# seagochen/unet-segment-pytorch

Hardware: NVIDIA B200
Metric: AttentionUNet 512^2 train images/sec (whole job; per GPU = value / n_gpus) (higher is better)
Workload: dtype bf16

## Files before the change

### include/unetb200.h

```cpp
#ifndef UNETB200_H
#define UNETB200_H
#include <stddef.h>
#include <stdint.h>

#ifdef __cplusplus
extern "C" {
#endif

#define UB2_OK 0
#define UB2_ERR_SHAPE (-1)
#define UB2_ERR_ALIGN (-2)
#define UB2_ERR_WORKSPACE (-3)
#define UB2_ERR_DRIVER (-4)
#define UB2_ERR_ARCH (-5)

int ub2_version(void);
int ub2_num_sms(void);
int ub2_set_conv_mode(int mode);
int ub2_last_conv_variant(void);


int ub2_conv_fwd(const void* in0, int ld_in0, int C0, const void* in1, int ld_in1, int C1,
                 const void* wgt, void* out0, int ld0, void* out1, int ld1, int split, int N, int H,
                 int W, int Cout, int taps, const float* scale, const float* shift, int relu,
                 int accumulate, double* stats, int stats_rows, int* stats_rows_used,
                 int bn_override, int grid_override, void* stream);

int ub2_conv_wgrad(const void* in0, int ld_in0, int C0, const void* in1, int ld_in1, int C1,
                   const void* dy, int ld_dy, float* partial, int max_splits, int* splits_used,
                   int N, int H, int W, int Cout, int taps, int splits_override, void* stream);

int ub2_wgrad_reduce(float* partial, int splits, int Cout, int Cin, int taps, float* grad,
                     int accumulate, void* stream);

#define UB2_REDUCE_MAX_ITEMS 32
typedef struct Ub2ReduceItem {
  float* partial;
  float* grad;
  int splits, Cout, Cin, taps;
} Ub2ReduceItem;
int ub2_wgrad_reduce_multi(const Ub2ReduceItem* items, int n, int accumulate, void* stream);

int ub2_pack_conv_weight(const float* w, void* fwd, void* dgrad, int Cout, int Cin, int taps,
                         const float* out_scale, void* stream);
int ub2_pack_conv_weights_multi(const long long* desc, const int* blocks, int nblocks, void* stream);


int ub2_bn_finalize(const double* partials, int rows, int C, double count, const float* gamma,
                    const float* beta, float* running_mean, float* running_var, long long* nbt,
                    float momentum, float eps, float* scale, float* shift, float* mean, float* invstd,
                    void* stream);
int ub2_bn_eval_coeffs(const float* gamma, const float* beta, const float* running_mean,
                       const float* running_var, float eps, int C, float* scale, float* shift,
                       void* stream);
int ub2_bn_act(const void* y, int ld_y, const float* scale, const float* shift, void* a, int ld_a,
               void* pooled, int ld_p, unsigned char* pidx, int N, int H, int W, int C, int relu,
               void* stream);
int ub2_bn_bwd_rows(int N, int H, int W, int C, int pool);
int ub2_bn_bwd_reduce(const void* dA, int ld_da, const void* dP, int ld_dp, const unsigned char* pidx,
// ... 150 lines not shown
```

### unet-segment-pytorch_b200/csrc/capi_conv.cu

```cuda
#include "../../include/unetb200.h"
#include "conv.h"

using namespace ub2;

extern "C" {

int ub2_conv_fwd(const void* in0, int ld_in0, int C0, const void* in1, int ld_in1, int C1,
                 const void* wgt, void* out0, int ld0, void* out1, int ld1, int split, int N, int H,
                 int W, int Cout, int taps, const float* scale, const float* shift, int relu,
                 int accumulate, double* stats, int stats_rows, int* stats_rows_used,
                 int bn_override, int grid_override, void* stream) {
  ConvFwdArgs a{};
  a.in0 = in0; a.in1 = in1; a.wgt = wgt; a.out0 = out0; a.out1 = out1;
  a.scale = scale; a.shift = shift; a.stats = stats; a.grid_used = stats_rows_used;
  a.N = N; a.H = H; a.W = W; a.C0 = C0; a.C1 = C1; a.Cout = Cout; a.taps = taps;
  a.ld_in0 = ld_in0; a.ld_in1 = ld_in1; a.ld0 = ld0; a.ld1 = ld1; a.split = split;
  a.accumulate = accumulate; a.relu = relu; a.stats_rows = stats_rows;
  a.bn_override = bn_override; a.grid_override = grid_override;
  return conv_fwd_launch(a, static_cast<cudaStream_t>(stream));
}

int ub2_conv_fwd_tf32(const float* in0, int ld_in0, int C0, const float* in1, int ld_in1, int C1,
                      const float* wgt, float* out, int ld_out, int N, int H, int W, int Cout, int taps,
                      const float* scale, const float* shift, int relu, int exact_out, void* stream) {
  ConvFwdArgs a{};
  a.in0 = in0; a.in1 = in1; a.wgt = wgt; a.out0 = out;
  a.scale = scale; a.shift = shift; a.relu = relu;
  a.N = N; a.H = H; a.W = W; a.C0 = C0; a.C1 = C1; a.Cout = Cout; a.taps = taps;
  a.ld_in0 = ld_in0; a.ld_in1 = ld_in1; a.ld0 = ld_out;
  a.tf32 = exact_out ? 2 : 1;
  return conv_fwd_launch(a, static_cast<cudaStream_t>(stream));
}

int ub2_conv_wgrad(const void* in0, int ld_in0, int C0, const void* in1, int ld_in1, int C1,
                   const void* dy, int ld_dy, float* partial, int max_splits, int* splits_used,
                   int N, int H, int W, int Cout, int taps, int splits_override, void* stream) {
  ConvWgradArgs a{};
  a.in0 = in0; a.in1 = in1; a.dy = dy; a.partial = partial; a.splits_used = splits_used;
  a.N = N; a.H = H; a.W = W; a.C0 = C0; a.C1 = C1; a.Cout = Cout; a.taps = taps;
  a.ld_in0 = ld_in0; a.ld_in1 = ld_in1; a.ld_dy = ld_dy;
  a.max_splits = max_splits; a.splits_override = splits_override;
  return conv_wgrad_launch(a, static_cast<cudaStream_t>(stream));
}

int ub2_num_sms(void) { return num_sms(); }

int ub2_last_conv_variant(void) { return last_variant(); }

int ub2_set_conv_mode(int mode) {
  conv_set_mode(mode);
  return 0;
}

}
```

### unet-segment-pytorch_b200/csrc/conv.h

```cpp
#pragma once
#include <cuda.h>
#include <cuda_bf16.h>
#include <cuda_runtime.h>
#include <stddef.h>
#include <stdint.h>
#include <stdlib.h>

#define UB2_ERR_SHAPE (-1)
#define UB2_ERR_ALIGN (-2)
#define UB2_ERR_WORKSPACE (-3)
#define UB2_ERR_DRIVER (-4)
#define UB2_ERR_ARCH (-5)

namespace ub2 {

struct ConvFwdArgs {
  const void* in0;
  const void* in1;
  const void* wgt;
  void* out0;
  void* out1;
  const float* scale;
  const float* shift;
  double* stats;
  int* grid_used;
  int N, H, W, C0, C1, Cout, taps;
  int ld_in0, ld_in1, ld0, ld1, split;
  int accumulate, relu;
  int stats_rows;
  int bn_override, grid_override;
  int tf32;
};

struct ConvFwdParams {
  int N, H, W, C0, C1, Cout, taps, kc;
  int BW, BH, BI, tiles_w, tiles_h, tiles_n;
  int BN, n_tiles, stages, stage_bytes, tmem_cols;
  __nv_bfloat16* out0;
  __nv_bfloat16* out1;
  int ld0, ld1, split, accumulate, relu;
  int wide_store;
  int tf32;
  const float* scale;
  const float* shift;
  double* stats;
  int R, segs_w, blocks_h, a_bytes, b_stage_bytes, b_stages;
};

int conv_fwd_launch(const ConvFwdArgs& a, cudaStream_t stream);
int conv_halo_launch(const ConvFwdArgs& a, cudaStream_t stream);
void conv_set_mode(int mode);

struct ConvWgradArgs {
  const void* in0;
  const void* in1;
  const void* dy;
  float* partial;
  int* splits_used;
  int N, H, W, C0, C1, Cout, taps;
  int ld_in0, ld_in1, ld_dy;
  int max_splits;
  int splits_override;
};

struct ConvWgradParams {
  int N, H, W, C0, C1, Cout, taps, mc;
  int BW, BH, BI, chunks_w, chunks_h, chunks_n;
  int BN, n_tiles, m_tiles, splits, stages, stage_bytes, tmem_cols;
  int a_sub_bytes, b_sub_bytes, a_bytes;
  float* partial;
};

int conv_wgrad_launch(const ConvWgradArgs& a, cudaStream_t stream);

int make_tmap_nhwc(CUtensorMap* m, const void* base, int N, int H, int W, int C, int ld,
                   const uint32_t box[4], int swizzle_bytes, int elem_bytes = 2);
int make_tmap_2d(CUtensorMap* m, const void* base, uint64_t cols, uint64_t rows, uint64_t ld,
                 uint32_t bc, uint32_t br, int swizzle_bytes, int elem_bytes = 2);
int num_sms();
inline int cap_clusters(int occupancy_clusters) { const int c = num_sms() / 2; return occupancy_clusters < c ? occupancy_clusters : c; }
inline int wgrad_smem_budget() {
  static const int kb = [] { const char* e = getenv("UB2_WGRAD_SMEM_KB"); int v = e ? atoi(e) : 163; return v < 64 ? 64 : (v > 227 ? 227 : v); }();
  return kb * 1024;
// ... 19 lines not shown
```

### unet-segment-pytorch_b200/csrc/conv_fwd.cu

```cuda
#include "launch.cuh"
#include <cstdlib>
#include "conv.h"
#include "conv_epilogue.cuh"
#include "ptx.cuh"

namespace ub2 {

static constexpr int kMaxStages = 8;
static constexpr int kEpiWarps = 8;
static constexpr int kThreads = 64 + 32 * kEpiWarps;
static constexpr int kATileBytes = 128 * 64 * 2;

struct FwdSmemHeader {
  uint64_t full[kMaxStages];
  uint64_t empty[kMaxStages];
  uint64_t tmem_full[2];
  uint64_t tmem_empty[2];
  uint32_t tmem_base;
  uint32_t pad;
};

template <int TAPS, bool ACC, bool TF32>
__global__ void __launch_bounds__(kThreads, 1)
conv_fwd_kernel(const __grid_constant__ CUtensorMap tmA0, const __grid_constant__ CUtensorMap tmA1,
// ... 147 lines not shown
      const int as = it & 1;
      mbar_wait(&hdr->tmem_full[as], (it >> 1) & 1);
      tc_fence_after();
      for (int j = grp; j < nchunks; j += 2) {
        epi_chunk<ACC, TF32>(p, tmem_base + (static_cast<uint32_t>(q * 32) << 16) + as * bn_cols + j * 32,
                       n0 + j * 32, n0 + BN, valid, pix, lane, want_stats, my_stats, acc_s, acc_q);
      }
      tc_fence_before();
      __syncwarp();
      if (lane == 0) mbar_arrive(&hdr->tmem_empty[as]);
    }
    if (want_stats)
      epi_finish<ACC, 32 * kEpiWarps>(p, s_stats, my_stats, lane, grp, nchunks, threadIdx.x - 64, acc_s, acc_q);
  }

  tc_fence_before();
  __syncthreads();
  if (warp == 1) {
    tc_fence_after();
    tmem_dealloc(tmem_base, p.tmem_cols);
  }
}


static int pow2_floor(int x) {
  int r = 1;
  while (r * 2 <= x) r *= 2;
  return r;
}

int conv_fwd2_launch(const ConvFwdArgs& a, cudaStream_t stream);

int conv_fwd_launch(const ConvFwdArgs& a, cudaStream_t stream) {
  if (!a.tf32) {
    const int rc = conv_halo_launch(a, stream);
    if (rc != 1) return rc;
  }
  {
    const int rc = conv_fwd2_launch(a, stream);
    if (rc != 1) return rc;
  }
  const int Ctot = a.C0 + a.C1;
  const int esz = a.tf32 ? 4 : 2;
  if (a.taps != 1 && a.taps != 9) return UB2_ERR_SHAPE;
  if (a.N <= 0 || a.H <= 0 || a.W <= 0 || a.C0 <= 0 || a.C1 < 0) return UB2_ERR_SHAPE;
  if (Ctot % 16 != 0 || a.C0 % 16 != 0 || a.Cout % 16 != 0) return UB2_ERR_SHAPE;
  if (a.ld_in0 % 8 != 0 || (a.C1 > 0 && a.ld_in1 % 8 != 0) || a.ld0 % 8 != 0) return UB2_ERR_ALIGN;
  if (a.tf32 && (a.stats != nullptr || a.accumulate || a.out1 != nullptr)) return UB2_ERR_SHAPE;
  int kc = 128 / esz;
  while (a.C0 % kc != 0 || Ctot % kc != 0) kc /= 2;

  ConvFwdParams p{};
  p.N = a.N; p.H = a.H; p.W = a.W;
  p.C0 = a.C0; p.C1 = a.C1; p.Cout = a.Cout;
  p.taps = a.taps; p.kc = kc;
  p.BW = pow2_floor(a.W < 128 ? a.W : 128);
  p.BH = pow2_floor(a.H < 128 / p.BW ? a.H : 128 / p.BW);
  p.BI = 128 / (p.BW * p.BH);
  p.tiles_w = (a.W + p.BW - 1) / p.BW;
  p.tiles_h = (a.H + p.BH - 1) / p.BH;
  p.tiles_n = (a.N + p.BI - 1) / p.BI;
  int BN = a.Cout <= 256 ? a.Cout : 256;
  const int split = (a.out1 != nullptr) ? a.split : (1 << 30);
  if (a.out1 != nullptr) {
    if (a.split % 8 != 0 || a.ld1 % 8 != 0) return UB2_ERR_ALIGN;
  }
// ... 90 lines not shown
```

### unet-segment-pytorch_b200/csrc/gate.cu

```cuda
#include "launch.cuh"
#include "../../include/unetb200.h"
#include "conv.h"
#include "resample.cuh"
#include "vec.cuh"

#include <cstdlib>
#include <mutex>
#include <utility>
#include <vector>

namespace ub2 {

static constexpr int kGateThreads = 256;
static constexpr int kMaxG = 2;

struct GateGeom {
  int N, H, W, C, cgs, tpp, slots;
  int pixels;
  int wt, ht;
  LowRes lr;
};
static constexpr int kGateStrip = 16;

static int gate_tpp(int cgs) {
// ... 496 lines not shown
#pragma unroll
      for (int k = 0; k < 8; ++k) v.v[k] *= a;
      store8(out + static_cast<size_t>(pixv[u]) * ld_out + cgv[u] * 8, v);
      if (cgv[u] == 0 && a_out != nullptr) a_out[pixv[u]] = a;
    }
  }
}

template <int G>
__global__ void __launch_bounds__(kGateThreads)
gate_bwd_a_kernel(const __nv_bfloat16* __restrict__ dout, int ld_do, const __nv_bfloat16* __restrict__ x,
                  int ld_x, const float* __restrict__ a, const float* __restrict__ psi_raw,
                  __nv_bfloat16* __restrict__ dx, int ld_dx, float* __restrict__ dpsin,
                  double* partials, GateGeom g) {
  pdl_trigger();
  pdl_wait();
  __shared__ float smem[kGateThreads / 32];
  float st[2] = {0.f, 0.f};
  GATE_PIXEL_LOOP(g) {
    GATE_PIX(g)
    const float av = pv ? __ldg(a + pix) : 0.f;
    float dot = 0.f;
#pragma unroll
    for (int gi = 0; gi < G; ++gi) {
      const int cg = j + gi * g.tpp;
      if (pv && cg < g.cgs) {
        F8 d = load8_stream(dout + static_cast<size_t>(pix) * ld_do + cg * 8);
        const F8 xv = load8_stream(x + static_cast<size_t>(pix) * ld_x + cg * 8);
#pragma unroll
        for (int k = 0; k < 8; ++k) {
          dot = fmaf(d.v[k], xv.v[k], dot);
          d.v[k] *= av;
        }
        store8(dx + static_cast<size_t>(pix) * ld_dx + cg * 8, d);
      }
    }
    dot = group_sum(dot, g.tpp);
    if (pv && j == 0) {
      const float dn = dot * av * (1.f - av);
      dpsin[pix] = dn;
      st[0] += dn;
      st[1] = fmaf(dn, __ldg(psi_raw + pix), st[1]);
    }
  }
  block_reduce_scalars<2>(st, partials + static_cast<size_t>(blockIdx.x) * 2, smem);
}

template <int G, int QR>
__global__ void __launch_bounds__(kGateThreads, G == 1 ? UB2_GATE_BWD_S_BLOCKS : 1)
gate_bwd_s_kernel(const float* __restrict__ dpsin, const float* __restrict__ psi_raw,
                  const float* __restrict__ coef_psi, const __nv_bfloat16* __restrict__ q, int ld_q,
                  const __nv_bfloat16* __restrict__ xp, int ld_xp, const float* __restrict__ sg,
                  const float* __restrict__ hg, const float* __restrict__ sx,
                  const float* __restrict__ hx, const float* __restrict__ wpsi,
                  __nv_bfloat16* __restrict__ ds, int ld_ds, double* partials, GateGeom g) {
  pdl_trigger();
  pdl_wait();
  __shared__ float smem[kGateThreads * 8];
  const float cA = __ldg(coef_psi), cB = __ldg(coef_psi + 1), cC = __ldg(coef_psi + 2);
  float acc[G][4][8];
#pragma unroll
  for (int a = 0; a < G; ++a)
#pragma unroll
    for (int b = 0; b < 4; ++b)
#pragma unroll
      for (int k = 0; k < 8; ++k) acc[a][b][k] = 0.f;
  typedef Strip<G, QR, 1, 2> S_t;
// ... 297 lines not shown
```

### unet-segment-pytorch_b200/csrc/ptx.cuh

```cuda
#pragma once
#include <cuda.h>
#include <cuda_bf16.h>
#include <cuda_runtime.h>
#include <stdint.h>
#include <stdio.h>

namespace ub2 {

__device__ __forceinline__ uint32_t smem_u32(const void* p) {
  return static_cast<uint32_t>(__cvta_generic_to_shared(p));
}

__device__ __forceinline__ bool elect_one() {
  uint32_t pred;
  asm volatile(
      "{\n\t.reg .pred P;\n\t"
      "elect.sync _|P, 0xffffffff;\n\t"
      "selp.u32 %0, 1, 0, P;\n\t}\n"
      : "=r"(pred));
  return pred != 0;
}

__device__ __forceinline__ void mbar_init(uint64_t* bar, uint32_t count) {
  asm volatile("mbarrier.init.shared::cta.b64 [%0], %1;" ::"r"(smem_u32(bar)), "r"(count));
// ... 22 lines not shown
}
__device__ __forceinline__ void mbar_wait(uint64_t* bar, uint32_t parity) {
  uint32_t spins = 0;
  while (!mbar_try_wait(bar, parity)) {
    if (++spins > (1u << 26)) {
      printf("ub2: mbarrier timeout block %d thread %d\n", (int)blockIdx.x, (int)threadIdx.x);
      __trap();
    }
  }
}

__device__ __forceinline__ void tma_prefetch_desc(const CUtensorMap* m) {
  asm volatile("prefetch.tensormap [%0];" ::"l"(reinterpret_cast<uint64_t>(m)) : "memory");
}
__device__ __forceinline__ void tma_load_2d(void* dst, const CUtensorMap* m, uint64_t* bar, int c0,
                                            int c1) {
  asm volatile(
      "cp.async.bulk.tensor.2d.shared::cluster.global.mbarrier::complete_tx::bytes"
      " [%0], [%1, {%3, %4}], [%2];"
      :
      : "r"(smem_u32(dst)), "l"(reinterpret_cast<uint64_t>(m)), "r"(smem_u32(bar)), "r"(c0),
        "r"(c1)
      : "memory");
}
__device__ __forceinline__ void tma_load_4d(void* dst, const CUtensorMap* m, uint64_t* bar, int c0,
                                            int c1, int c2, int c3) {
  asm volatile(
      "cp.async.bulk.tensor.4d.shared::cluster.global.mbarrier::complete_tx::bytes"
      " [%0], [%1, {%3, %4, %5, %6}], [%2];"
      :
      : "r"(smem_u32(dst)), "l"(reinterpret_cast<uint64_t>(m)), "r"(smem_u32(bar)), "r"(c0),
        "r"(c1), "r"(c2), "r"(c3)
      : "memory");
}

__device__ __forceinline__ void tc_fence_before() {
  asm volatile("tcgen05.fence::before_thread_sync;" ::: "memory");
}
__device__ __forceinline__ void tc_fence_after() {
  asm volatile("tcgen05.fence::after_thread_sync;" ::: "memory");
}
__device__ __forceinline__ void tmem_alloc(uint32_t* dst_smem, uint32_t ncols) {
  asm volatile("tcgen05.alloc.cta_group::1.sync.aligned.shared::cta.b32 [%0], %1;" ::"r"(
                   smem_u32(dst_smem)),
               "r"(ncols)
               : "memory");
  asm volatile("tcgen05.relinquish_alloc_permit.cta_group::1.sync.aligned;" ::: "memory");
}
__device__ __forceinline__ void tmem_dealloc(uint32_t addr, uint32_t ncols) {
  asm volatile("tcgen05.dealloc.cta_group::1.sync.aligned.b32 %0, %1;" ::"r"(addr), "r"(ncols)
               : "memory");
}
__device__ __forceinline__ void umma_bf16(uint32_t tmem_d, uint64_t desc_a, uint64_t desc_b,
                                          uint32_t idesc, uint32_t accumulate) {
  asm volatile(
      "{\n\t.reg .pred p;\n\t"
      "setp.ne.b32 p, %4, 0;\n\t"
      "tcgen05.mma.cta_group::1.kind::f16 [%0], %1, %2, %3, p;\n\t}\n"
      :
      : "r"(tmem_d), "l"(desc_a), "l"(desc_b), "r"(idesc), "r"(accumulate)
      : "memory");
}
__device__ __forceinline__ void umma_tf32(uint32_t tmem_d, uint64_t desc_a, uint64_t desc_b,
                                          uint32_t idesc, uint32_t accumulate) {
  asm volatile(
      "{\n\t.reg .pred p;\n\t"
      "setp.ne.b32 p, %4, 0;\n\t"
      "tcgen05.mma.cta_group::1.kind::tf32 [%0], %1, %2, %3, p;\n\t}\n"
      :
      : "r"(tmem_d), "l"(desc_a), "l"(desc_b), "r"(idesc), "r"(accumulate)
      : "memory");
}
__device__ __forceinline__ void umma_commit(uint64_t* bar) {
  asm volatile("tcgen05.commit.cta_group::1.mbarrier::arrive::one.shared::cluster.b64 [%0];" ::"r"(
                   smem_u32(bar))
               : "memory");
}
__device__ __forceinline__ void tmem_ld32(uint32_t taddr, uint32_t (&v)[32]) {
  asm volatile(
      "tcgen05.ld.sync.aligned.32x32b.x32.b32 "
      "{%0, %1, %2, %3, %4, %5, %6, %7, %8, %9, %10, %11, %12, %13, %14, %15, "
      "%16, %17, %18, %19, %20, %21, %22, %23, %24, %25, %26, %27, %28, %29, %30, %31}, [%32];"
      : "=r"(v[0]), "=r"(v[1]), "=r"(v[2]), "=r"(v[3]), "=r"(v[4]), "=r"(v[5]), "=r"(v[6]),
        "=r"(v[7]), "=r"(v[8]), "=r"(v[9]), "=r"(v[10]), "=r"(v[11]), "=r"(v[12]), "=r"(v[13]),
        "=r"(v[14]), "=r"(v[15]), "=r"(v[16]), "=r"(v[17]), "=r"(v[18]), "=r"(v[19]), "=r"(v[20]),
        "=r"(v[21]), "=r"(v[22]), "=r"(v[23]), "=r"(v[24]), "=r"(v[25]), "=r"(v[26]), "=r"(v[27]),
        "=r"(v[28]), "=r"(v[29]), "=r"(v[30]), "=r"(v[31])
      : "r"(taddr)
      : "memory");
}
__device__ __forceinline__ void tmem_ld_wait() {
  asm volatile("tcgen05.wait::ld.sync.aligned;" ::: "memory");
}

__device__ __forceinline__ uint64_t make_smem_desc(uint32_t saddr, uint32_t lbo_bytes,
                                                   uint32_t sbo_bytes, uint32_t layout_type) {
  uint64_t d = 0;
  d |= static_cast<uint64_t>((saddr & 0x3FFFF) >> 4);
  d |= static_cast<uint64_t>((lbo_bytes >> 4) & 0x3FFF) << 16;
  d |= static_cast<uint64_t>((sbo_bytes >> 4) & 0x3FFF) << 32;
  d |= static_cast<uint64_t>(1) << 46;
  d |= static_cast<uint64_t>(layout_type & 7) << 61;
  return d;
}
__host__ __device__ __forceinline__ uint32_t make_idesc_bf16(uint32_t M, uint32_t N,
                                                             uint32_t a_mn_major,
                                                             uint32_t b_mn_major) {
  return (1u << 4) | (1u << 7) | (1u << 10) | (a_mn_major << 15) | (b_mn_major << 16) |
         ((N >> 3) << 17) | ((M >> 4) << 24);
}

__host__ __device__ __forceinline__ uint32_t make_idesc_tf32(uint32_t M, uint32_t N) {
  return (1u << 4) | (2u << 7) | (2u << 10) | ((N >> 3) << 17) | ((M >> 4) << 24);
}

__device__ __forceinline__ float tf32_round(float x) {
  uint32_t r;
  asm("cvt.rna.tf32.f32 %0, %1;" : "=r"(r) : "f"(x));
  return __uint_as_float(r);
}
__device__ __forceinline__ uint32_t pack_bf16x2(float lo, float hi) {
  __nv_bfloat162 v = __floats2bfloat162_rn(lo, hi);
  return *reinterpret_cast<uint32_t*>(&v);
// ... 15 lines not shown
```

### unet-segment-pytorch_b200/unet/kernels.py

```python
from __future__ import annotations

import ctypes

import torch

from . import _C
from ._C import byref, c_double, c_float, c_int, c_longlong, ptr, stream

BF16 = torch.bfloat16
F32 = torch.float32
F64 = torch.float64

_SMS = None


def _nbytes(*tensors) -> int:
    return sum(t.numel() * t.element_size() for t in tensors if t is not None)


def num_sms() -> int:
    global _SMS
    if _SMS is None:
        _SMS = int(_C.lib().ub2_num_sms())
    return _SMS
# ... 257 lines not shown
    return partials


def gate_psi(q, xp, sg, hg, sx, hx, wpsi, stats=True):
    n, hin, win, ci, ld_q = _nhwc(q)
    _, h, w, _, ld_xp = _nhwc(xp)
    psi = torch.empty((n, h, w), device=q.device, dtype=F32)
    rows = gate_strip_rows(n, h, w, ci)
    partials = torch.empty((rows, 2, 1), device=q.device, dtype=F64) if stats else None
    _C.call("ub2_gate_psi", ptr(q), ld_q, ptr(xp), ld_xp, ptr(sg), ptr(hg), ptr(sx), ptr(hx), ptr(wpsi),
            ptr(psi), ptr(partials), rows, n, hin, win, h, w, ci, stream(), work=(0.0, _nbytes(q, xp, psi)))
    return psi, partials


def gate_fused_eval(q, xp, x, sg, hg, sx, hx, wpsi, spsi, hpsi):
    n, hin, win, ci, ld_q = _nhwc(q)
    _, h, w, _, ld_xp = _nhwc(xp)
    _, _, _, cx, ld_x = _nhwc(x)
    out = empty_nhwc(n, h, w, cx, x.device)
    _C.call("ub2_gate_fused_eval", ptr(q), ld_q, ptr(xp), ld_xp, ptr(x), ld_x, ptr(sg), ptr(hg), ptr(sx), ptr(hx), ptr(wpsi),
            ptr(spsi), ptr(hpsi), ptr(out), cx, n, hin, win, h, w, ci, cx, stream(), work=(0.0, _nbytes(q, xp, x, out)))
    return out


def gate_apply(psi, spsi, hpsi, x, save_a=True):
    n, h, w, cx, ld = _nhwc(x)
    out = empty_nhwc(n, h, w, cx, x.device)
    a = torch.empty((n, h, w), device=x.device, dtype=F32) if save_a else None
    _C.call("ub2_gate_apply", ptr(psi), ptr(spsi), ptr(hpsi), ptr(x), ld, ptr(out), cx, ptr(a), n, h, w,
            cx, stream(), work=(0.0, _nbytes(psi, x, out, a)))
    return out, a


def gate_bwd_a(dout, x, a, psi):
    n, h, w, cx, ld_x = _nhwc(x)
    ld_do = _nhwc(dout)[4]
    dx = empty_nhwc(n, h, w, cx, x.device)
    dpsin = torch.empty((n, h, w), device=x.device, dtype=F32)
    rows = gate_rows(n, h, w, cx)
    partials = torch.empty((rows, 2, 1), device=x.device, dtype=F64)
    _C.call("ub2_gate_bwd_a", ptr(dout), ld_do, ptr(x), ld_x, ptr(a), ptr(psi), ptr(dx), cx, ptr(dpsin),
            ptr(partials), rows, n, h, w, cx, stream(), work=(0.0, _nbytes(dout, x, a, psi, dx, dpsin)))
    return dx, dpsin, partials


def gate_bwd_s(dpsin, psi, coef_psi, q, xp, sg, hg, sx, hx, wpsi):
    n, hin, win, ci, ld_q = _nhwc(q)
    _, h, w, _, ld_xp = _nhwc(xp)
    ds = empty_nhwc(n, h, w, ci, q.device)
    rows = gate_strip_rows(n, h, w, ci)
    partials = torch.empty((rows, 4, ci), device=q.device, dtype=F64)
    _C.call("ub2_gate_bwd_s", ptr(dpsin), ptr(psi), ptr(coef_psi), ptr(q), ld_q, ptr(xp), ld_xp, ptr(sg),
            ptr(hg), ptr(sx), ptr(hx), ptr(wpsi), ptr(ds), ci, ptr(partials), rows, n, hin, win, h, w, ci,
            stream(), work=(0.0, _nbytes(dpsin, psi, q, xp, ds)))
    return ds, partials


def gate_bwd_finalize(partials, count, gamma_x, mean_x, invstd_x, gamma_g, mean_g, invstd_g, frozen=False,
                      targets=None):
    rows, _, ci = partials.shape
    grads = targets if targets is not None else torch.zeros((5, ci), device=partials.device, dtype=F32)
    coef = torch.empty((6, ci), device=partials.device, dtype=F32)
    _C.call("ub2_gate_bwd_finalize", ptr(partials), rows, ci, c_double(float(count)), ptr(gamma_x),
            ptr(mean_x), ptr(invstd_x), ptr(gamma_g), ptr(mean_g), ptr(invstd_g), int(frozen), ptr(grads[0]),
            ptr(grads[1]),
            ptr(grads[2]), ptr(grads[3]), ptr(grads[4]), ptr(coef), stream())
    return grads, coef


def gate_bwd_xg(ds, xp, q, coef):
    n, hin, win, ci, ld_q = _nhwc(q)
    _, h, w, _, ld_xp = _nhwc(xp)
    dxp = empty_nhwc(n, h, w, ci, q.device)
    dgup = empty_nhwc(n, h, w, ci, q.device)
    _C.call("ub2_gate_bwd_xg", ptr(ds), _nhwc(ds)[4], ptr(xp), ld_xp, ptr(q), ld_q, ptr(coef), ptr(dxp), ci,
            ptr(dgup), ci, n, hin, win, h, w, ci, stream(), work=(0.0, _nbytes(ds, xp, q, dxp, dgup)))
# ... 191 lines not shown
```

### unet-segment-pytorch_b200/unet/ops.py

```python
from __future__ import annotations

import torch

from . import kernels as K

BF16 = torch.bfloat16


GRAD_SINK = None


def _grad_targets(*params):
    if GRAD_SINK is None:
        return None
    out = []
    for p in params:
        if not getattr(p, "is_leaf", False):
            return None
        g = getattr(p, "grad", None)
        if (g is None or g.dtype != torch.float32 or not g.is_contiguous()
                or g.numel() != p.numel() or g.device != p.device):
            return None
        out.append(g)
    return out
# ... 259 lines not shown
            sx, hx, mx, ix = _bn_train_coeffs(st_x, count, bn_x)
        else:
            xp = K.conv_fwd(xn, wxf, 1)
            sg, hg, mg, ig = _bn_frozen_coeffs(bn_g)
            sx, hx, mx, ix = _bn_frozen_coeffs(bn_x)
        if not batch and not need_grad and cx == 2 * wpsi.numel():
            sp, hp, _, _ = _bn_frozen_coeffs(bn_p)
            return from_nhwc(K.gate_fused_eval(q, xp, xn, sg, hg, sx, hx, wpsi, sp, hp))
        psi, st_p = K.gate_psi(q, xp, sg, hg, sx, hx, wpsi, stats=batch)
        if batch:
            sp, hp, mp, ip = _bn_train_coeffs(st_p, count, bn_p)
        else:
            sp, hp, mp, ip = _bn_frozen_coeffs(bn_p)
        out, a = K.gate_apply(psi, sp, hp, xn, save_a=need_grad)
        if need_grad:
            ctx.save_for_backward(gn, xn, q, xp, psi, a, sg, hg, mg, ig, sx, hx, mx, ix, mp, ip, wgd, wxd,
                                  wpsi, gam_g, gam_x, gam_p)
            ctx.meta = (w_g.shape, w_x.shape, w_psi.shape, batch)
            ctx.params = (w_g, w_x, w_psi, gam_g, bet_g, gam_x, bet_x, gam_p, bet_p)
        return from_nhwc(out)

    @staticmethod
    def backward(ctx, dout):
        (gn, xn, q, xp, psi, a, sg, hg, mg, ig, sx, hx, mx, ix, mp, ip, wgd, wxd, wpsi, gam_g, gam_x,
         gam_p) = ctx.saved_tensors
        sh_g, sh_x, sh_p, batch = ctx.meta
        n, h, w, cx = xn.shape
        _, hin, win, cg = gn.shape
        ci = q.shape[3]
        count = n * h * w
        d = to_nhwc(dout)
        p_wg, p_wx, p_wpsi, p_gg, p_bg, p_gx, p_bx, p_gp, p_bp = ctx.params
        direct = _grad_targets(*ctx.params) if all(ctx.needs_input_grad[2:11]) else None
        dx, dpsin, part = K.gate_bwd_a(d, xn, a, psi)
        if direct is not None:
            t_wg, t_wx, t_wpsi, t_gg, t_bg, t_gx, t_bx, t_gp, t_bp = direct
            _, _, coef_p = K.bn_bwd_finalize(part, count, gam_p, mp, ip, frozen=not batch, dgamma=t_gp, dbeta=t_bp)
        else:
            dgam_p, dbet_p, coef_p = K.bn_bwd_finalize(part, count, gam_p, mp, ip, frozen=not batch)
        ds, part2 = K.gate_bwd_s(dpsin, psi, coef_p, q, xp, sg, hg, sx, hx, wpsi)
        grads, coef = K.gate_bwd_finalize(part2, count, gam_x, mx, ix, gam_g, mg, ig, frozen=not batch,
                                          targets=[t_gx, t_bx, t_gg, t_bg, t_wpsi] if direct is not None else None)
        dxp, dgup = K.gate_bwd_xg(ds, xp, q, coef)
        dq = K.upsample_bwd(dgup, hin, win, h, w)
        if direct is not None:
            _reduce_into(p_wx, K.conv_wgrad(xn, dxp, 1), ci, cx, 1, t_wx)
            _reduce_into(p_wg, K.conv_wgrad(gn, dq, 1), ci, cg, 1, t_wg)
        else:
            gw_x = torch.empty(sh_x, device=d.device, dtype=torch.float32)
            K.wgrad_reduce(K.conv_wgrad(xn, dxp, 1), ci, cx, 1, gw_x)
            gw_g = torch.empty(sh_g, device=d.device, dtype=torch.float32)
            K.wgrad_reduce(K.conv_wgrad(gn, dq, 1), ci, cg, 1, gw_g)
        K.conv_fwd(dxp, wxd, 1, out=dx, accumulate=True)
        dg = K.conv_fwd(dq, wgd, 1)
        if direct is not None:
            _grads_done(*ctx.params[2:])
            return (from_nhwc(dg), from_nhwc(dx)) + (None,) * 12
        return (from_nhwc(dg), from_nhwc(dx), gw_g, gw_x, grads[4].reshape(sh_p), grads[2], grads[3],
                grads[0], grads[1], dgam_p, dbet_p, None, None, None)


class OutConvFn(torch.autograd.Function):

    @staticmethod
    def forward(ctx, x, weight, bias):
        a = to_nhwc(x)
        if any(ctx.needs_input_grad):
            ctx.save_for_backward(a, weight)
            ctx.params = (weight, bias)
        return K.outc_fwd(a, weight.reshape(weight.shape[0], -1), bias)

    @staticmethod
    def backward(ctx, dlogits):
        a, weight = ctx.saved_tensors
        direct = _grad_targets(*ctx.params) if ctx.needs_input_grad[1] and ctx.needs_input_grad[2] else None
        da, dw, db = K.outc_bwd(dlogits.contiguous().float(), a, weight.reshape(weight.shape[0], -1),
                                need_da=ctx.needs_input_grad[0],
                                dw=direct[0] if direct is not None else None,
                                db=direct[1] if direct is not None else None)
        da = from_nhwc(da) if da is not None else None
        if direct is not None:
            _grads_done(*ctx.params)
            return da, None, None
        return da, dw.reshape(weight.shape), db


# ... 99 lines not shown
```

Baseline: 593.0.

## Add dedicated 1x1 projection conv kernel with fused gated residual in attention backward

Adds a persistent tcgen05/TMA kernel specialised for 1x1 convolutions (pixel-major GEMM with weights resident in shared memory, pipelined A loads, double-buffered TMEM accumulators and TMA stores). It handles plain, accumulate and BN-stats modes, and all eligible 1x1 forward convs are routed to it first. The attention-gate backward also gains a fused gated mode that computes dx = dout*a + conv(dxp) in one kernel, so gate_bwd_a no longer writes dx and conv_fwd no longer re-reads it. This removes a full activation round-trip and gives small-K 1x1 GEMMs a better-suited kernel. The cost is a large new code path with its own synchronisation and a risk of being slower than the existing halo kernel for some shapes.

```diff
diff --git a/include/unetb200.h b/include/unetb200.h
--- a/include/unetb200.h
+++ b/include/unetb200.h
@@ -25,6 +25,10 @@
                  int W, int Cout, int taps, const float* scale, const float* shift, int relu,
                  int accumulate, double* stats, int stats_rows, int* stats_rows_used,
                  int bn_override, int grid_override, void* stream);
+
+int ub2_conv_proj_gated(const void* in, int ld_in, int Cin, const void* wgt, const void* dout, int ld_do,
+                        const float* a, void* out, int ld_out, long long pixels, int Cout, void* stream);
+int ub2_conv_proj_gated_ok(long long pixels, int Cin, int Cout);
 
 int ub2_conv_wgrad(const void* in0, int ld_in0, int C0, const void* in1, int ld_in1, int C1,
                    const void* dy, int ld_dy, float* partial, int max_splits, int* splits_used,
diff --git a/unet-segment-pytorch_b200/csrc/capi_conv.cu b/unet-segment-pytorch_b200/csrc/capi_conv.cu
--- a/unet-segment-pytorch_b200/csrc/capi_conv.cu
+++ b/unet-segment-pytorch_b200/csrc/capi_conv.cu
@@ -43,6 +43,14 @@
   return conv_wgrad_launch(a, static_cast<cudaStream_t>(stream));
 }
 
+int ub2_conv_proj_gated(const void* in, int ld_in, int Cin, const void* wgt, const void* dout, int ld_do,
+                        const float* a, void* out, int ld_out, long long pixels, int Cout, void* stream) {
+  return conv_proj_gated_launch(in, ld_in, wgt, dout, ld_do, a, out, ld_out, pixels, Cin, Cout,
+                                static_cast<cudaStream_t>(stream));
+}
+
+int ub2_conv_proj_gated_ok(long long pixels, int Cin, int Cout) { return conv_proj_gated_ok(pixels, Cin, Cout); }
+
 int ub2_num_sms(void) { return num_sms(); }
 
 int ub2_last_conv_variant(void) { return last_variant(); }
diff --git a/unet-segment-pytorch_b200/csrc/conv.h b/unet-segment-pytorch_b200/csrc/conv.h
--- a/unet-segment-pytorch_b200/csrc/conv.h
+++ b/unet-segment-pytorch_b200/csrc/conv.h
@@ -49,6 +49,10 @@
 
 int conv_fwd_launch(const ConvFwdArgs& a, cudaStream_t stream);
 int conv_halo_launch(const ConvFwdArgs& a, cudaStream_t stream);
+int conv_proj_launch(const ConvFwdArgs& a, cudaStream_t stream);
+int conv_proj_gated_ok(long long pixels, int Cin, int Cout);
+int conv_proj_gated_launch(const void* in, int ld_in, const void* wgt, const void* dout, int ld_do, const float* a,
+                           void* out, int ld_out, long long pixels, int Cin, int Cout, cudaStream_t stream);
 void conv_set_mode(int mode);
 
 struct ConvWgradArgs {
diff --git a/unet-segment-pytorch_b200/csrc/conv_fwd.cu b/unet-segment-pytorch_b200/csrc/conv_fwd.cu
--- a/unet-segment-pytorch_b200/csrc/conv_fwd.cu
+++ b/unet-segment-pytorch_b200/csrc/conv_fwd.cu
@@ -203,6 +203,10 @@
 int conv_fwd2_launch(const ConvFwdArgs& a, cudaStream_t stream);
 
 int conv_fwd_launch(const ConvFwdArgs& a, cudaStream_t stream) {
+  if (a.taps == 1) {
+    const int rc = conv_proj_launch(a, stream);
+    if (rc != 1) return rc;
+  }
   if (!a.tf32) {
     const int rc = conv_halo_launch(a, stream);
     if (rc != 1) return rc;
diff --git a/unet-segment-pytorch_b200/csrc/conv_proj.cu b/unet-segment-pytorch_b200/csrc/conv_proj.cu
--- /dev/null
+++ b/unet-segment-pytorch_b200/csrc/conv_proj.cu
@@ -0,0 +1,493 @@
+#include "launch.cuh"
+#include <cstdlib>
+#include "conv.h"
+#include "ptx.cuh"
+
+namespace ub2 {
+
+namespace {
+
+constexpr int kPStages = 12;
+constexpr int kPAddSlots = 4;
+constexpr int kPMaxBufs = 8;
+constexpr int kPEpiWarps = 8;
+constexpr int kPThreads = 64 + 32 * kPEpiWarps;
+
+enum { kPlain = 0, kAccumulate = 1, kGated = 2 };
+
+struct ProjHeader {
+  uint64_t full[kPStages];
+  uint64_t empty[kPStages];
+  uint64_t add_full[kPAddSlots];
+  uint64_t add_empty[kPAddSlots];
+  uint64_t tmem_full[kPMaxBufs];
+  uint64_t tmem_empty[kPMaxBufs];
+  uint64_t wbar;
+  uint32_t tmem_base;
+  uint32_t pad;
+};
+
+struct ProjParams {
+  int P, Cin, Cout, kc, tiles;
+  int stages, add_slots, nbufs, nstg, tmem_cols;
+  int a_bytes, add_bytes;
+  int w_off, a_off, add_off, stg_off, hdr_off;
+  double* stats;
+};
+
+__device__ __forceinline__ uint32_t swz(int row, int chunk, int row_bytes) {
+  const int sw = ((row * row_bytes) >> 7) & (row_bytes / 16 - 1);
+  return static_cast<uint32_t>(row * row_bytes + ((chunk ^ sw) << 4));
+}
+
+__device__ __forceinline__ float butterfly16(float (&v)[16], int lane) {
+#pragma unroll
+  for (int k = 0; k < 16; ++k) v[k] += __shfl_xor_sync(0xffffffffu, v[k], 16);
+#pragma unroll
+  for (int m = 8; m >= 1; m >>= 1) {
+    const bool up = (lane & m) != 0;
+#pragma unroll
+    for (int k = 0; k < m; ++k) {
+      const float keep = up ? v[k + m] : v[k];
+      const float send = up ? v[k] : v[k + m];
+      v[k] = keep + __shfl_xor_sync(0xffffffffu, send, m);
+    }
+  }
+  return v[0];
+}
+
+enum { kNoStats = 0, kTileStats = 1, kRunStats = 2 };
+
+template <int MODE, int STATS>
+__global__ void __launch_bounds__(kPThreads, 1)
+conv_proj_kernel(const __grid_constant__ CUtensorMap tmA, const __grid_constant__ CUtensorMap tmW,
+                 const __grid_constant__ CUtensorMap tmO, const __grid_constant__ CUtensorMap tmD,
+                 const __grid_constant__ CUtensorMap tmG, const ProjParams p) {
+  pdl_trigger();
+  extern __shared__ __align__(1024) uint8_t smem_raw[];
+  uint8_t* base = reinterpret_cast<uint8_t*>((reinterpret_cast<uintptr_t>(smem_raw) + 1023) &
+                                             ~static_cast<uintptr_t>(1023));
+  uint8_t* s_w = base + p.w_off;
+  uint8_t* s_a = base + p.a_off;
+  uint8_t* s_add = base + p.add_off;
+  uint8_t* s_stg = base + p.stg_off;
+  ProjHeader* hdr = reinterpret_cast<ProjHeader*>(base + p.hdr_off);
+  float* s_stats = reinterpret_cast<float*>(hdr + 1);
+  constexpr bool ADD = MODE != kPlain;
+
+  const int warp = threadIdx.x >> 5;
+  const int lane = threadIdx.x & 31;
+  const int Cout = p.Cout;
+  const int kchunks = p.Cin / p.kc;
+  const int stages = p.stages;
+
+  if (warp == 0 && lane == 0) {
+    tma_prefetch_desc(&tmA);
+    tma_prefetch_desc(&tmW);
+    tma_prefetch_desc(&tmO);
+    if (ADD) tma_prefetch_desc(&tmD);
+    if (MODE == kGated) tma_prefetch_desc(&tmG);
+    for (int i = 0; i < stages; ++i) {
+      mbar_init(&hdr->full[i], 1);
+      mbar_init(&hdr->empty[i], 1);
+    }
+    for (int i = 0; i < p.add_slots; ++i) {
+      mbar_init(&hdr->add_full[i], 1);
+      mbar_init(&hdr->add_empty[i], kPEpiWarps);
+    }
+    for (int i = 0; i < p.nbufs; ++i) {
+      mbar_init(&hdr->tmem_full[i], 1);
+      mbar_init(&hdr->tmem_empty[i], kPEpiWarps);
+    }
+    mbar_init(&hdr->wbar, 1);
+    fence_mbar_init();
+  }
+  if (warp == 1) tmem_alloc(&hdr->tmem_base, p.tmem_cols);
+  if (STATS != kNoStats && warp >= 2) {
+    for (int i = threadIdx.x - 64; i < 4 * 2 * Cout; i += 32 * kPEpiWarps) s_stats[i] = 0.f;
+  }
+  tc_fence_before();
+  __syncthreads();
+  tc_fence_after();
+  const uint32_t tmem_base = hdr->tmem_base;
+  pdl_wait();
+
+  if (warp == 0) {
+    const uint32_t w_chunk = static_cast<uint32_t>(Cout) * p.kc * 2;
+    if (elect_one()) {
+      mbar_expect_tx(&hdr->wbar, w_chunk * kchunks);
+      for (int kb = 0; kb < kchunks; ++kb) tma_load_2d(s_w + kb * w_chunk, &tmW, &hdr->wbar, kb * p.kc, 0);
+    }
+    const int acw = Cout < 64 ? Cout : 64;
+    const int ablk = 128 * acw * 2;
+    int stage = 0, slot = 0;
+    uint32_t phase = 0, aphase = 0;
+    for (int t = blockIdx.x; t < p.tiles; t += gridDim.x) {
+      const int r0 = t * 128;
+      if (ADD) {
+        mbar_wait(&hdr->add_empty[slot], aphase ^ 1);
+        if (elect_one()) {
+          uint8_t* dst = s_add + slot * p.add_bytes;
+          mbar_expect_tx(&hdr->add_full[slot], static_cast<uint32_t>(128 * Cout * 2 + (MODE == kGated ? 512 : 0)));
+          for (int c = 0; c < Cout; c += acw) tma_load_2d(dst + (c / acw) * ablk, &tmD, &hdr->add_full[slot], c, r0);
+          if (MODE == kGated) tma_load_2d(dst + 128 * Cout * 2, &tmG, &hdr->add_full[slot], r0, 0);
+        }
+        if (++slot == p.add_slots) {
+          slot = 0;
+          aphase ^= 1;
+        }
+      }
+      for (int kb = 0; kb < kchunks; ++kb) {
+        mbar_wait(&hdr->empty[stage], phase ^ 1);
+        if (elect_one()) {
+          mbar_expect_tx(&hdr->full[stage], static_cast<uint32_t>(p.a_bytes));
+          tma_load_2d(s_a + stage * p.a_bytes, &tmA, &hdr->full[stage], kb * p.kc, r0);
+        }
+        if (++stage == stages) {
+          stage = 0;
+          phase ^= 1;
+        }
+      }
+    }
+  } else if (warp == 1) {
+    const uint32_t idesc = make_idesc_bf16(128, Cout, 0, 0);
+    const uint32_t row_bytes = static_cast<uint32_t>(p.kc) * 2u;
+    const uint32_t ltype = (row_bytes == 128) ? 2u : (row_bytes == 64) ? 4u : 6u;
+    const uint32_t desc_hi = ((8u * row_bytes) >> 4) | (1u << 14) | (ltype << 29);
+    const uint32_t a_lo0 = ((smem_u32(s_a) & 0x3FFFFu) >> 4) | (1u << 16);
+    const uint32_t w_lo0 = ((smem_u32(s_w) & 0x3FFFFu) >> 4) | (1u << 16);
+    const uint32_t a_inc = static_cast<uint32_t>(p.a_bytes) >> 4;
+    const uint32_t w_inc = (static_cast<uint32_t>(Cout) * row_bytes) >> 4;
+    const int kinner = static_cast<int>(row_bytes / 32);
+    mbar_wait(&hdr->wbar, 0);
+    tc_fence_after();
+    int stage = 0, buf = 0;
+    uint32_t phase = 0, bphase = 0;
+    for (int t = blockIdx.x; t < p.tiles; t += gridDim.x) {
+      mbar_wait(&hdr->tmem_empty[buf], bphase ^ 1);
+      tc_fence_after();
+      const uint32_t d_tmem = tmem_base + buf * Cout;
+      for (int kb = 0; kb < kchunks; ++kb) {
+        mbar_wait(&hdr->full[stage], phase);
+        tc_fence_after();
+        if (elect_one()) {
+          const uint32_t a_lo = a_lo0 + stage * a_inc;
+          const uint32_t b_lo = w_lo0 + kb * w_inc;
+          for (int k = 0; k < kinner; ++k) {
+            const uint64_t da = (static_cast<uint64_t>(desc_hi) << 32) | (a_lo + 2 * k);
+            const uint64_t db = (static_cast<uint64_t>(desc_hi) << 32) | (b_lo + 2 * k);
+            umma_bf16(d_tmem, da, db, idesc, (kb | k) != 0);
+          }
+          umma_commit(&hdr->empty[stage]);
+          if (kb == kchunks - 1) umma_commit(&hdr->tmem_full[buf]);
+        }
+        __syncwarp();
+        if (++stage == stages) {
+          stage = 0;
+          phase ^= 1;
+        }
+      }
+      if (++buf == p.nbufs) {
+        buf = 0;
+        bphase ^= 1;
+      }
+    }
+  } else {
+    const int q = warp & 3;
+    const int ew = warp - 2;
+    const int grp = ew >> 2;
+    const int row = q * 32 + lane;
+    const int half = Cout / 2;
+    const int cw = half < 64 ? half : 64;
+    const int srow = cw * 2;
+    const int acw = Cout < 64 ? Cout : 64;
+    const int arow = acw * 2;
+    const int stg_bytes = 32 * Cout;
+    float* my_stats = s_stats + q * 2 * Cout;
+    constexpr int RN = STATS == kRunStats ? 16 : 1;
+    float run_s[2][RN], run_q[2][RN];
+#pragma unroll
+    for (int i = 0; i < RN; ++i) run_s[0][i] = run_s[1][i] = run_q[0][i] = run_q[1][i] = 0.f;
+    int buf = 0, slot = 0, it = 0;
+    uint32_t bphase = 0, aphase = 0;
+    for (int t = blockIdx.x; t < p.tiles; t += gridDim.x, ++it) {
+      mbar_wait(&hdr->tmem_full[buf], bphase);
+      tc_fence_after();
+      const uint8_t* add = s_add + slot * p.add_bytes;
+      if (ADD) mbar_wait(&hdr->add_full[slot], aphase);
+      float av = 0.f;
+      if (MODE == kGated) av = reinterpret_cast<const float*>(add + 128 * Cout * 2)[row];
+      uint8_t* stg = s_stg + (ew * p.nstg + (it % p.nstg)) * stg_bytes;
+      if (lane == 0) {
+        if (p.nstg == 2) bulk_wait_read<1>();
+        else bulk_wait_read<0>();
+      }
+      __syncwarp();
+      for (int c = 0; c < half; c += 16) {
+        const int col = grp * half + c;
+        uint32_t raw[16];
+        tmem_ld16(tmem_base + (static_cast<uint32_t>(q * 32) << 16) + buf * Cout + col, raw);
+        tmem_ld_wait();
+        float v[16];
+#pragma unroll
+        for (int i = 0; i < 16; ++i) v[i] = __uint_as_float(raw[i]);
+        if (ADD) {
+          const uint8_t* ab = add + (col / acw) * (128 * arow);
+          const int ch = (col % acw) >> 3;
+          const uint4 u[2] = {*reinterpret_cast<const uint4*>(ab + swz(row, ch, arow)),
+                              *reinterpret_cast<const uint4*>(ab + swz(row, ch + 1, arow))};
+#pragma unroll
+          for (int h = 0; h < 2; ++h) {
+            const uint32_t w4[4] = {u[h].x, u[h].y, u[h].z, u[h].w};
+#pragma unroll
+            for (int k = 0; k < 4; ++k) {
+              if (MODE == kAccumulate) {
+                v[h * 8 + 2 * k] += bf16_lo(w4[k]);
+                v[h * 8 + 2 * k + 1] += bf16_hi(w4[k]);
+              } else {
+                v[h * 8 + 2 * k] += bf16_round(bf16_lo(w4[k]) * av);
+                v[h * 8 + 2 * k + 1] += bf16_round(bf16_hi(w4[k]) * av);
+              }
+            }
+          }
+        }
+        uint4 o[2];
+#pragma unroll
+        for (int h = 0; h < 2; ++h) {
+          o[h].x = pack_bf16x2(v[h * 8 + 0], v[h * 8 + 1]);
+          o[h].y = pack_bf16x2(v[h * 8 + 2], v[h * 8 + 3]);
+          o[h].z = pack_bf16x2(v[h * 8 + 4], v[h * 8 + 5]);
+          o[h].w = pack_bf16x2(v[h * 8 + 6], v[h * 8 + 7]);
+        }
+        uint8_t* sb = stg + (c / cw) * (32 * srow);
+        const int sch = (c % cw) >> 3;
+        *reinterpret_cast<uint4*>(sb + swz(lane, sch, srow)) = o[0];
+        *reinterpret_cast<uint4*>(sb + swz(lane, sch + 1, srow)) = o[1];
+        if (STATS != kNoStats) {
+          float s[16], sq[16];
+#pragma unroll
+          for (int h = 0; h < 2; ++h) {
+            const uint32_t w4[4] = {o[h].x, o[h].y, o[h].z, o[h].w};
+#pragma unroll
+            for (int k = 0; k < 4; ++k) {
+              s[h * 8 + 2 * k] = bf16_lo(w4[k]);
+              s[h * 8 + 2 * k + 1] = bf16_hi(w4[k]);
+            }
+          }
+          if (STATS == kRunStats) {
+#pragma unroll
+            for (int i = 0; i < RN; ++i) {
+              if (c == 0) {
+                run_s[0][i] += s[i];
+                run_q[0][i] = fmaf(s[i], s[i], run_q[0][i]);
+              } else {
+                run_s[1][i] += s[i];
+                run_q[1][i] = fmaf(s[i], s[i], run_q[1][i]);
+              }
+            }
+          } else {
+#pragma unroll
+            for (int i = 0; i < 16; ++i) sq[i] = s[i] * s[i];
+            const float s1 = butterfly16(s, lane);
+            const float s2 = butterfly16(sq, lane);
+            if (lane < 16) {
+              my_stats[col + lane] += s1;
+              my_stats[Cout + col + lane] += s2;
+            }
+          }
+        }
+      }
+      tc_fence_before();
+      fence_proxy_async_smem();
+      __syncwarp();
+      if (lane == 0) {
+        mbar_arrive(&hdr->tmem_empty[buf]);
+        if (ADD) mbar_arrive(&hdr->add_empty[slot]);
+        for (int c = 0; c < half; c += cw)
+          tma_store_2d(&tmO, stg + (c / cw) * (32 * srow), grp * half + c, t * 128 + q * 32);
+        bulk_commit();
+      }
+      if (++buf == p.nbufs) {
+        buf = 0;
+        bphase ^= 1;
+      }
+      if (ADD && ++slot == p.add_slots) {
+        slot = 0;
+        aphase ^= 1;
+      }
+    }
+    if (lane == 0) bulk_wait_all();
+    if (STATS == kRunStats) {
+#pragma unroll
+      for (int ci = 0; ci < 2; ++ci) {
+        if (ci * 16 < half) {
+          float a[16], b[16];
+#pragma unroll
+          for (int i = 0; i < 16; ++i) {
+            a[i] = run_s[ci][i < RN ? i : 0];
+            b[i] = run_q[ci][i < RN ? i : 0];
+          }
+          const float s1 = butterfly16(a, lane);
+          const float s2 = butterfly16(b, lane);
+          if (lane < 16) {
+            my_stats[grp * half + ci * 16 + lane] = s1;
+            my_stats[Cout + grp * half + ci * 16 + lane] = s2;
+          }
+        }
+      }
+    }
+    if (STATS != kNoStats) {
+      asm volatile("bar.sync 1, %0;" ::"n"(32 * kPEpiWarps) : "memory");
+      for (int c = threadIdx.x - 64; c < Cout; c += 32 * kPEpiWarps) {
+        double s1 = 0.0, s2 = 0.0;
+        for (int e = 0; e < 4; ++e) {
+          s1 += static_cast<double>(s_stats[e * 2 * Cout + c]);
+          s2 += static_cast<double>(s_stats[e * 2 * Cout + Cout + c]);
+        }
+        p.stats[(static_cast<size_t>(blockIdx.x) * 2 + 0) * Cout + c] = s1;
+        p.stats[(static_cast<size_t>(blockIdx.x) * 2 + 1) * Cout + c] = s2;
+      }
+    }
+  }
+
+  tc_fence_before();
+  __syncthreads();
+  if (warp == 1) {
+    tc_fence_after();
+    tmem_dealloc(tmem_base, p.tmem_cols);
+  }
+}
+
+constexpr int kSmemLimit = 227 * 1024;
+
+bool proj_plan(int P, int Cin, int Cout, int mode, bool stats, ProjParams* p) {
+  static const bool enabled = [] { const char* e = getenv("UB2_GATE_PROJ"); return e == nullptr || atoi(e) != 0; }();
+  if (!enabled) return false;
+  if (P <= 0 || Cin <= 0 || Cin % 16 != 0 || Cout <= 0 || Cout % 32 != 0 || Cout > 256) return false;
+  *p = ProjParams{};
+  p->P = P; p->Cin = Cin; p->Cout = Cout;
+  p->kc = Cin % 64 == 0 ? 64 : (Cin % 32 == 0 ? 32 : 16);
+  p->tiles = (P + 127) / 128;
+  p->a_bytes = 128 * p->kc * 2;
+  p->add_bytes = mode == kPlain ? 0 : ((128 * Cout * 2 + (mode == kGated ? 512 : 0) + 1023) & ~1023);
+  const int w_bytes = Cin * Cout * 2;
+  const int stg = 32 * Cout;
+  const int fixed = 1024 + static_cast<int>(sizeof(ProjHeader)) + (stats ? 4 * 2 * Cout * 4 : 0) + w_bytes;
+  const int tries[3][2] = {{2, kPAddSlots}, {2, 2}, {1, 2}};
+  for (const auto& tr : tries) {
+    const int add_slots = mode == kPlain ? 0 : tr[1];
+    const int rest = kSmemLimit - fixed - kPEpiWarps * tr[0] * stg - add_slots * p->add_bytes;
+    int stages = rest / p->a_bytes;
+    if (stages > kPStages) stages = kPStages;
+    if (stages >= 2) {
+      p->nstg = tr[0];
+      p->add_slots = add_slots;
+      p->stages = stages;
+      break;
+    }
+  }
+  if (p->stages < 2) return false;
+  int nbufs = 256 / Cout;
+  if (nbufs > kPMaxBufs) nbufs = kPMaxBufs;
+  if (nbufs < 2) nbufs = 2;
+  p->nbufs = nbufs;
+  int cols = 32;
+  while (cols < nbufs * Cout) cols *= 2;
+  p->tmem_cols = cols;
+  p->w_off = 0;
+  p->a_off = w_bytes;
+  p->add_off = p->a_off + p->stages * p->a_bytes;
+  p->stg_off = p->add_off + p->add_slots * p->add_bytes;
+  p->hdr_off = p->stg_off + kPEpiWarps * p->nstg * stg;
+  return true;
+}
+
+size_t proj_smem(const ProjParams& p, bool stats) {
+  return 1024 + static_cast<size_t>(p.hdr_off) + sizeof(ProjHeader) + (stats ? 4 * 2 * p.Cout * 4 : 0);
+}
+
+int set_smem_attrs() {
+  static PerDevice<bool> done_pd;
+  bool& done = done_pd.ref();
+  if (done) return 0;
+  const auto attr = cudaFuncAttributeMaxDynamicSharedMemorySize;
+  cudaError_t e = cudaFuncSetAttribute(conv_proj_kernel<kPlain, kNoStats>, attr, kSmemLimit);
+  if (e == cudaSuccess) e = cudaFuncSetAttribute(conv_proj_kernel<kPlain, kTileStats>, attr, kSmemLimit);
+  if (e == cudaSuccess) e = cudaFuncSetAttribute(conv_proj_kernel<kPlain, kRunStats>, attr, kSmemLimit);
+  if (e == cudaSuccess) e = cudaFuncSetAttribute(conv_proj_kernel<kAccumulate, kNoStats>, attr, kSmemLimit);
+  if (e == cudaSuccess) e = cudaFuncSetAttribute(conv_proj_kernel<kGated, kNoStats>, attr, kSmemLimit);
+  if (e != cudaSuccess) return static_cast<int>(e);
+  done = true;
+  return 0;
+}
+
+int proj_launch(int mode, const void* in, int ld_in, const void* wgt, void* out, int ld_out, const void* dout,
+                int ld_do, const float* a, double* stats, int stats_rows, int* grid_used, long long pixels, int Cin,
+                int Cout, cudaStream_t stream) {
+  if (pixels >= (1ll << 31) - 128) return 1;
+  const int P = static_cast<int>(pixels);
+  ProjParams p;
+  if (!proj_plan(P, Cin, Cout, mode, stats != nullptr, &p)) return 1;
+  p.stats = stats;
+  const int half = Cout / 2;
+  const uint32_t cw = static_cast<uint32_t>(half < 64 ? half : 64);
+  const uint32_t acw = static_cast<uint32_t>(Cout < 64 ? Cout : 64);
+  CUtensorMap tmA, tmW, tmO, tmD, tmG;
+  int rc = make_tmap_2d(&tmA, in, Cin, P, ld_in, p.kc, 128, p.kc * 2);
+  if (!rc) rc = make_tmap_2d(&tmW, wgt, Cin, Cout, Cin, p.kc, Cout, p.kc * 2);
+  if (!rc) rc = make_tmap_2d(&tmO, out, Cout, P, ld_out, cw, 32, cw * 2);
+  if (rc) return rc;
+  tmD = tmG = tmO;
+  if (mode == kAccumulate) rc = make_tmap_2d(&tmD, out, Cout, P, ld_out, acw, 128, acw * 2);
+  if (mode == kGated) {
+    rc = make_tmap_2d(&tmD, dout, Cout, P, ld_do, acw, 128, acw * 2);
+    if (!rc) rc = make_tmap_2d(&tmG, a, P, 1, (static_cast<uint64_t>(P) + 3) & ~3ull, 128, 1, 0, 4);
+  }
+  if (rc) return rc;
+  int grid = num_sms();
+  if (grid > p.tiles) grid = p.tiles;
+  if (stats && grid > stats_rows) return UB2_ERR_WORKSPACE;
+  const size_t smem = proj_smem(p, stats != nullptr);
+  if ((rc = set_smem_attrs())) return rc;
+  note_variant(5);
+  if (mode == kGated)
+    launch(conv_proj_kernel<kGated, kNoStats>, grid, kPThreads, smem, stream, tmA, tmW, tmO, tmD, tmG, p);
+  else if (mode == kAccumulate)
+    launch(conv_proj_kernel<kAccumulate, kNoStats>, grid, kPThreads, smem, stream, tmA, tmW, tmO, tmD, tmG, p);
+  else if (stats && Cout <= 64)
+    launch(conv_proj_kernel<kPlain, kRunStats>, grid, kPThreads, smem, stream, tmA, tmW, tmO, tmD, tmG, p);
+  else if (stats)
+    launch(conv_proj_kernel<kPlain, kTileStats>, grid, kPThreads, smem, stream, tmA, tmW, tmO, tmD, tmG, p);
+  else
+    launch(conv_proj_kernel<kPlain, kNoStats>, grid, kPThreads, smem, stream, tmA, tmW, tmO, tmD, tmG, p);
+  const cudaError_t e = cudaGetLastError();
+  if (e != cudaSuccess) return static_cast<int>(e);
+  if (grid_used) *grid_used = grid;
+  return 0;
+}
+
+}
+
+int conv_proj_launch(const ConvFwdArgs& a, cudaStream_t stream) {
+  if (a.tf32 || a.taps != 1 || a.C1 != 0 || a.out1 != nullptr || a.scale != nullptr || a.relu ||
+      a.bn_override > 0 || a.grid_override > 0)
+    return 1;
+  if (a.N <= 0 || a.H <= 0 || a.W <= 0) return 1;
+  return proj_launch(a.accumulate ? kAccumulate : kPlain, a.in0, a.ld_in0, a.wgt, a.out0, a.ld0, nullptr, 0, nullptr,
+                     a.stats, a.stats_rows, a.grid_used, static_cast<long long>(a.N) * a.H * a.W, a.C0, a.Cout,
+                     stream);
+}
+
+int conv_proj_gated_ok(long long pixels, int Cin, int Cout) {
+  ProjParams p;
+  return pixels > 0 && pixels < (1ll << 31) - 128 && proj_plan(static_cast<int>(pixels), Cin, Cout, kGated, false, &p);
+}
+
+int conv_proj_gated_launch(const void* in, int ld_in, const void* wgt, const void* dout, int ld_do, const float* a,
+                           void* out, int ld_out, long long pixels, int Cin, int Cout, cudaStream_t stream) {
+  const int rc = proj_launch(kGated, in, ld_in, wgt, out, ld_out, dout, ld_do, a, nullptr, 0, nullptr, pixels, Cin,
+                             Cout, stream);
+  return rc == 1 ? UB2_ERR_SHAPE : rc;
+}
+
+}
diff --git a/unet-segment-pytorch_b200/csrc/gate.cu b/unet-segment-pytorch_b200/csrc/gate.cu
--- a/unet-segment-pytorch_b200/csrc/gate.cu
+++ b/unet-segment-pytorch_b200/csrc/gate.cu
@@ -552,7 +552,7 @@
           dot = fmaf(d.v[k], xv.v[k], dot);
           d.v[k] *= av;
         }
-        store8(dx + static_cast<size_t>(pix) * ld_dx + cg * 8, d);
+        if (dx != nullptr) store8(dx + static_cast<size_t>(pix) * ld_dx + cg * 8, d);
       }
     }
     dot = group_sum(dot, g.tpp);
diff --git a/unet-segment-pytorch_b200/csrc/ptx.cuh b/unet-segment-pytorch_b200/csrc/ptx.cuh
--- a/unet-segment-pytorch_b200/csrc/ptx.cuh
+++ b/unet-segment-pytorch_b200/csrc/ptx.cuh
@@ -78,6 +78,22 @@
       : "r"(smem_u32(dst)), "l"(reinterpret_cast<uint64_t>(m)), "r"(smem_u32(bar)), "r"(c0),
         "r"(c1), "r"(c2), "r"(c3)
       : "memory");
+}
+
+__device__ __forceinline__ void tma_store_2d(const CUtensorMap* m, const void* src, int c0, int c1) {
+  asm volatile("cp.async.bulk.tensor.2d.global.shared::cta.bulk_group [%0, {%2, %3}], [%1];" ::"l"(
+                   reinterpret_cast<uint64_t>(m)),
+               "r"(smem_u32(src)), "r"(c0), "r"(c1)
+               : "memory");
+}
+__device__ __forceinline__ void bulk_commit() { asm volatile("cp.async.bulk.commit_group;" ::: "memory"); }
+template <int N>
+__device__ __forceinline__ void bulk_wait_read() {
+  asm volatile("cp.async.bulk.wait_group.read %0;" ::"n"(N) : "memory");
+}
+__device__ __forceinline__ void bulk_wait_all() { asm volatile("cp.async.bulk.wait_group 0;" ::: "memory"); }
+__device__ __forceinline__ void fence_proxy_async_smem() {
+  asm volatile("fence.proxy.async.shared::cta;" ::: "memory");
 }
 
 __device__ __forceinline__ void tc_fence_before() {
@@ -135,6 +151,16 @@
       : "r"(taddr)
       : "memory");
 }
+__device__ __forceinline__ void tmem_ld16(uint32_t taddr, uint32_t (&v)[16]) {
+  asm volatile(
+      "tcgen05.ld.sync.aligned.32x32b.x16.b32 "
+      "{%0, %1, %2, %3, %4, %5, %6, %7, %8, %9, %10, %11, %12, %13, %14, %15}, [%16];"
+      : "=r"(v[0]), "=r"(v[1]), "=r"(v[2]), "=r"(v[3]), "=r"(v[4]), "=r"(v[5]), "=r"(v[6]),
+        "=r"(v[7]), "=r"(v[8]), "=r"(v[9]), "=r"(v[10]), "=r"(v[11]), "=r"(v[12]), "=r"(v[13]),
+        "=r"(v[14]), "=r"(v[15])
+      : "r"(taddr)
+      : "memory");
+}
 __device__ __forceinline__ void tmem_ld_wait() {
   asm volatile("tcgen05.wait::ld.sync.aligned;" ::: "memory");
 }
diff --git a/unet-segment-pytorch_b200/unet/kernels.py b/unet-segment-pytorch_b200/unet/kernels.py
--- a/unet-segment-pytorch_b200/unet/kernels.py
+++ b/unet-segment-pytorch_b200/unet/kernels.py
@@ -313,16 +313,34 @@
     return out, a
 
 
-def gate_bwd_a(dout, x, a, psi):
+def gate_bwd_a(dout, x, a, psi, want_dx=True):
     n, h, w, cx, ld_x = _nhwc(x)
     ld_do = _nhwc(dout)[4]
-    dx = empty_nhwc(n, h, w, cx, x.device)
+    dx = empty_nhwc(n, h, w, cx, x.device) if want_dx else None
     dpsin = torch.empty((n, h, w), device=x.device, dtype=F32)
     rows = gate_rows(n, h, w, cx)
     partials = torch.empty((rows, 2, 1), device=x.device, dtype=F64)
     _C.call("ub2_gate_bwd_a", ptr(dout), ld_do, ptr(x), ld_x, ptr(a), ptr(psi), ptr(dx), cx, ptr(dpsin),
             ptr(partials), rows, n, h, w, cx, stream(), work=(0.0, _nbytes(dout, x, a, psi, dx, dpsin)))
     return dx, dpsin, partials
+
+
+def conv_proj_gated_ok(pixels, cin, cout) -> bool:
+    return bool(_C.lib().ub2_conv_proj_gated_ok(c_longlong(pixels), cin, cout))
+
+
+def conv_proj_gated(dxp, wgt, dout, a, out=None):
+    n, h, w, cin, ld_in = _nhwc(dxp)
+    _, _, _, cout, ld_do = _nhwc(dout)
+    assert wgt.dtype == BF16 and wgt.is_contiguous() and wgt.numel() == cout * cin
+    assert a.dtype == F32 and a.is_contiguous() and a.numel() == n * h * w
+    if out is None:
+        out = empty_nhwc(n, h, w, cout, dxp.device)
+    ld_out = _nhwc(out)[4]
+    _C.call("ub2_conv_proj_gated", ptr(dxp), ld_in, cin, ptr(wgt), ptr(dout), ld_do, ptr(a), ptr(out), ld_out,
+            c_longlong(n * h * w), cout, stream(),
+            work=(2.0 * n * h * w * cout * cin, _nbytes(dxp, wgt, dout, a, out)))
+    return out
 
 
 def gate_bwd_s(dpsin, psi, coef_psi, q, xp, sg, hg, sx, hx, wpsi):
diff --git a/unet-segment-pytorch_b200/unet/ops.py b/unet-segment-pytorch_b200/unet/ops.py
--- a/unet-segment-pytorch_b200/unet/ops.py
+++ b/unet-segment-pytorch_b200/unet/ops.py
@@ -315,7 +315,8 @@
         d = to_nhwc(dout)
         p_wg, p_wx, p_wpsi, p_gg, p_bg, p_gx, p_bx, p_gp, p_bp = ctx.params
         direct = _grad_targets(*ctx.params) if all(ctx.needs_input_grad[2:11]) else None
-        dx, dpsin, part = K.gate_bwd_a(d, xn, a, psi)
+        gated = K.conv_proj_gated_ok(count, ci, cx)
+        dx, dpsin, part = K.gate_bwd_a(d, xn, a, psi, want_dx=not gated)
         if direct is not None:
             t_wg, t_wx, t_wpsi, t_gg, t_bg, t_gx, t_bx, t_gp, t_bp = direct
             _, _, coef_p = K.bn_bwd_finalize(part, count, gam_p, mp, ip, frozen=not batch, dgamma=t_gp, dbeta=t_bp)
@@ -334,7 +335,10 @@
             K.wgrad_reduce(K.conv_wgrad(xn, dxp, 1), ci, cx, 1, gw_x)
             gw_g = torch.empty(sh_g, device=d.device, dtype=torch.float32)
             K.wgrad_reduce(K.conv_wgrad(gn, dq, 1), ci, cg, 1, gw_g)
-        K.conv_fwd(dxp, wxd, 1, out=dx, accumulate=True)
+        if gated:
+            dx = K.conv_proj_gated(dxp, wxd, d, a)
+        else:
+            K.conv_fwd(dxp, wxd, 1, out=dx, accumulate=True)
         dg = K.conv_fwd(dq, wgd, 1)
         if direct is not None:
             _grads_done(*ctx.params[2:])
```

New measurement: 601.6, median of 6. 1.4% higher.
